# tomvanbraeckel/amv-codec-tools

Measured on AMD Instinct MI355X. Metric: AMV frames/sec/GPU (160x120 decode, bit-exact), higher is better.
Workload: dtype int32; 1 GPU; 160x120 AMV decode, 160000-frame synthetic stream per GPU, chunks resident in HBM; parallelism=frame-range x1, frames_per_gpu=160000, stream=seeded synthetic source (BASELINE.md section 4), every frame

## Files before the change

### amv-codec-tools_amd/csrc/amv_reconstruct.hip

```cpp
#include "amv_block_load.h"

namespace amv {

namespace {

struct __attribute__((aligned(4))) Px12 { uint32_t w[3]; };

constexpr int kRowsPerGroup = 4;

__device__ __forceinline__ int mad24(int x, int w, int c) {
    int d;
    asm("v_mad_i32_i24 %0, %1, %2, %3" : "=v"(d) : "v"(x), "s"(w), "v"(c));
    return d;
}

enum RowKind { kRowPlain, kRow0, kRow4 };

template <bool kColumn, RowKind kKind = kRowPlain>
__device__ __forceinline__ void idct8(int& v0, int& v1, int& v2, int& v3, int& v4, int& v5, int& v6, int& v7) {
    constexpr int W1 = 2841, W2 = 2676, W3 = 2408, W5 = 1609, W6 = 1108, W7 = 565;
    constexpr int kBias = kKind == kRow0 ? 128 + 8192 : 128;
    constexpr int kRound = kColumn ? 4 : 0;
    constexpr int kDown = kColumn ? 3 : 0;
    constexpr int kOut = kColumn ? 14 : 8;
    int a0 = kColumn ? v0 : v0 * 2048 + kBias, a1 = kColumn ? v4 : v4 * 2048;
    const int i2 = v6, i3 = v2, i4 = v1, i5 = v7, i6 = v5, i7 = v3;
    int t;
    int a4 = mad24(i4, W1, mad24(i5, W7, kRound)) >> kDown;
    int a5 = mad24(i4, W7, mad24(i5, -W1, kRound)) >> kDown;
    int a6 = mad24(i6, W5, mad24(i7, W3, kRound)) >> kDown;
    int a7 = mad24(i6, W3, mad24(i7, -W5, kRound)) >> kDown;
    t = a0 + a1;
    a0 -= a1;
    int a2 = mad24(i3, W6, mad24(i2, -W2, kRound)) >> kDown;
    int a3 = mad24(i3, W2, mad24(i2, W6, kRound)) >> kDown;
    a1 = a4 + a6;
    a4 -= a6;
    a6 = a5 + a7;
    a5 -= a7;
    a7 = t + a3;
    t -= a3;
    a3 = a0 + a2;
    a0 -= a2;
    a2 = (181 * (a4 + a5) + 128) >> 8;
    a4 = (181 * (a4 - a5) + 128) >> 8;
    v0 = a7 + a1;
    v1 = a3 + a2;
    v2 = a0 + a4;
    v3 = t + a6;
    v4 = t - a6;
    v5 = a0 - a4;
    v6 = a3 - a2;
    v7 = a7 - a1;
    if (kKind == kRowPlain) {
        v0 >>= kOut; v1 >>= kOut; v2 >>= kOut; v3 >>= kOut; v4 >>= kOut; v5 >>= kOut; v6 >>= kOut; v7 >>= kOut;
    } else {
        v0 &= ~255; v1 &= ~255; v2 &= ~255; v3 &= ~255; v4 &= ~255; v5 &= ~255; v6 &= ~255; v7 &= ~255;
    }
}

struct QuantWords { uint32_t w[2][16]; };
constexpr QuantWords pack_quant() {
    QuantWords q{};
    for (int i = 0; i < 64; ++i) {
        q.w[0][i >> 2] |= (uint32_t)kQuantLuma[i] << (8 * (i & 3));
        q.w[1][i >> 2] |= (uint32_t)kQuantChroma[i] << (8 * (i & 3));
    }
    return q;
}
__device__ const QuantWords kQuantWords = pack_quant();

__device__ __forceinline__ int clamp_iclp(int x) { return min(max(x, -256), 255); }

constexpr uint32_t pair16(int lo, int hi) { return ((uint32_t)lo & 0xffffu) | ((uint32_t)hi << 16); }
__device__ __forceinline__ uint32_t dot2_bias(uint32_t a, uint32_t w) {
    uint32_t d;
    asm("v_dot2_i32_i16 %0, %1, %2, %3" : "=v"(d) : "v"(a), "s"(w), "v"(32768u));
    return d;
}

__device__ __forceinline__ uint32_t sat_pair(uint32_t yy, uint32_t cc) {
    uint32_t sum, d;
    asm("v_pk_add_i16 %0, %1, %2" : "=v"(sum) : "v"(yy), "v"(cc));
    asm("v_sat_pk_u8_i16 %0, %1" : "=v"(d) : "v"(sum));
    return d;
}

}

template <bool kRound, int kRows>
__global__ __launch_bounds__(kWave * kRows) void amv_reconstruct_kernel(
    SyncSinks in, const uint32_t* __restrict__ nmcu_ok, uint32_t n, FrameSel sel,
    FrameGeom g, PieceMap pm, uint32_t flags, uint8_t* __restrict__ out) {
    constexpr uint32_t kPitchY = kSegMcus * 16, kPitchC = kSegMcus * 8;
    __shared__ __attribute__((aligned(16))) int16_t s_all[kRows][16 * kPitchY + 2 * 8 * kPitchC + 64];
    static_assert((16 * kPitchY + 2 * 8 * kPitchC) * 2 == kSegImageBytes, "the planes reuse the image");
    const uint32_t lane = threadIdx.x & 63u, wave = (uint32_t)__builtin_amdgcn_readfirstlane((int)(threadIdx.x >> 6));
    uint32_t item, row_group, seg;
    if (!locate_piece(pm, blockIdx.x, item, row_group, seg)) return;
    const uint32_t my = row_group * kRows + wave;
    if (my >= g.mcu_rows) return;
    int16_t* const s_mem = s_all[wave];
    int16_t* const s_y = s_mem;
    int16_t* const s_u = s_mem + 16 * kPitchY;
    int16_t* const s_v = s_u + 8 * kPitchC;
    uint8_t* const s_img = reinterpret_cast<uint8_t*>(s_mem);

    uint32_t qw[16];
    {
        const uint4* q4 = reinterpret_cast<const uint4*>(kQuantWords.w[lane % 6u >= 4u ? 1 : 0]);
#pragma unroll
        for (int i = 0; i < 4; ++i) {
            const uint4 q = q4[i];
            qw[4 * i] = q.x; qw[4 * i + 1] = q.y; qw[4 * i + 2] = q.z; qw[4 * i + 3] = q.w;
        }
    }
    do {
    uint32_t f, slot;
    if (!select_frame(sel, n, item, f, slot)) return;
    const Segment sg = segment_of(f, slot, nmcu_ok, g, pm.nseg, my, seg);
    const uint32_t m0 = sg.m0, cnt = sg.cnt, ok = sg.ok, mcu0 = sg.mcu0;

    uint32_t c[32];
    bool skip;
    if (load_segment_blocks(in, sg, kRound, g, lane, s_img, c, skip)) {
        const uint32_t m = lane / 6u, k6 = lane % 6u;
        const bool chroma = k6 >= 4u;
        int v[64];
#pragma unroll
        for (int nat = 0; nat < 64; ++nat) {
            const int scan = kScanOfNatural[nat];
            v[nat] = coef_at(c, scan) * (int)((qw[scan >> 2] >> (8 * (scan & 3))) & 255u);
        }
        if (!(flags & kFlagZigzagFixed))
            v[kAmvlibQuirkNatural] = coef_at(c, kAmvlibQuirkScan) * (int)((qw[kAmvlibQuirkScan >> 2] >> (8 * (kAmvlibQuirkScan & 3))) & 255u);
#pragma unroll
        for (int r = 0; r < 8; ++r) {
            if (r == 0) idct8<false, kRow0>(v[0], v[1], v[2], v[3], v[4], v[5], v[6], v[7]);
            else if (r == 4) idct8<false, kRow4>(v[32], v[33], v[34], v[35], v[36], v[37], v[38], v[39]);
            else idct8<false>(v[8 * r], v[8 * r + 1], v[8 * r + 2], v[8 * r + 3], v[8 * r + 4], v[8 * r + 5], v[8 * r + 6], v[8 * r + 7]);
        }
#pragma unroll
        for (int col = 0; col < 8; ++col)
            idct8<true>(v[col], v[8 + col], v[16 + col], v[24 + col], v[32 + col], v[40 + col], v[48 + col], v[56 + col]);
        int16_t* dst = chroma ? (k6 == 4u ? s_u : s_v) + m * 8u
                              : s_y + ((k6 >> 1) * 8u) * kPitchY + m * 16u + (k6 & 1u) * 8u;
        const uint32_t pitch = chroma ? kPitchC : kPitchY;
#pragma unroll
        for (int r = 0; r < 8; ++r) {
            uint32_t w[4];
#pragma unroll
            for (int q = 0; q < 4; ++q) {
                const int lo = clamp_iclp(v[8 * r + 2 * q]);
                const int hi = clamp_iclp(v[8 * r + 2 * q + 1]);
                w[q] = __builtin_amdgcn_perm((uint32_t)hi, (uint32_t)lo, 0x05040100u);
            }
            *reinterpret_cast<uint4*>(dst + r * pitch) = make_uint4(w[0], w[1], w[2], w[3]);
        }
    }
    if (skip) return;
    seg_sync();

    const uint32_t vr = min(16u, g.height - my * 16u);
    const uint32_t px = min(cnt * 16u, g.width - m0 * 16u);
    const uint32_t groups = cnt * 4u;
    const bool all_decoded = mcu0 + cnt <= ok;
    const uint32_t pairs = (vr + 1u) >> 1;
    const uint32_t step_i2 = kWave / groups, step_gi = kWave - step_i2 * groups;
    uint32_t i2 = lane / groups, gi = lane - i2 * groups;
    uint8_t* const frame = out + (uint64_t)f * g.frame_bytes;
    const uint32_t row0 = (g.height - 1u - my * 16u) * g.stride + m0 * 48u;
    for (; i2 < pairs; i2 += step_i2, gi += step_gi) {
        if (gi >= groups) { gi -= groups; ++i2; if (i2 >= pairs) break; }
        const uint32_t lc = gi * 4u;
        uint2 ya = *reinterpret_cast<const uint2*>(s_y + (2u * i2) * kPitchY + lc);
        uint2 yb = *reinterpret_cast<const uint2*>(s_y + (2u * i2 + 1u) * kPitchY + lc);
        uint32_t uu = *reinterpret_cast<const uint32_t*>(s_u + i2 * kPitchC + (lc >> 1));
        uint32_t vv = *reinterpret_cast<const uint32_t*>(s_v + i2 * kPitchC + (lc >> 1));
        if (!all_decoded && (mcu0 + (gi >> 2)) >= ok) {
            constexpr uint32_t kDark = 0xfc00fc00u;
            ya.x = ya.y = yb.x = yb.y = kDark;
            uu = vv = 0u;
        }
        uint32_t cr[2], cg[2], cb[2];
#pragma unroll
        for (int e = 0; e < 2; ++e) {
            const uint32_t uv = __builtin_amdgcn_perm(vv, uu, e ? 0x07060302u : 0x05040100u);
            const uint32_t r = dot2_bias(uv, pair16(18, 367));
            const uint32_t gg = dot2_bias(uv, pair16(-159, -220));
            const uint32_t b = dot2_bias(uv, pair16(411, -29));
            cr[e] = __builtin_amdgcn_perm(r, r, 0x02010201u);
            cg[e] = __builtin_amdgcn_perm(gg, gg, 0x02010201u);
            cb[e] = __builtin_amdgcn_perm(b, b, 0x02010201u);
        }
        if (lc >= px) continue;
        uint32_t off = row0 - 2u * i2 * g.stride + lc * 3u;
#pragma unroll
        for (int row = 0; row < 2; ++row) {
            const uint2 yy = row ? yb : ya;
            const uint32_t b01 = sat_pair(yy.x, cb[0]), g01 = sat_pair(yy.x, cg[0]), r01 = sat_pair(yy.x, cr[0]);
            const uint32_t b23 = sat_pair(yy.y, cb[1]), g23 = sat_pair(yy.y, cg[1]), r23 = sat_pair(yy.y, cr[1]);
            const uint32_t gr = g01 | (r01 << 16);
            const uint32_t bg = b23 | (g23 << 16);
            Px12 v;
            v.w[0] = __builtin_amdgcn_perm(gr, b01, 0x01060400u);
            v.w[1] = __builtin_amdgcn_perm(bg, gr, 0x06040301u);
            v.w[2] = __builtin_amdgcn_perm(bg, r23, 0x01070500u);
            if (2u * i2 + (uint32_t)row >= vr) break;
            if (lc + 4u <= px) {
                *reinterpret_cast<Px12*>(frame + off) = v;
            } else {
#pragma unroll
                for (uint32_t q = 0; q < 9u; ++q)
                    if (q < (px - lc) * 3u) frame[off + q] = (uint8_t)(v.w[q >> 2] >> (8u * (q & 3u)));
            }
            off -= g.stride;
        }
    }
    } while (next_item<kRound>(pm, item));
}

template <int kRows, class... Args>
static void launch_rows(const FrameGeom& g, Args... args) {
    launch_segments(amv_reconstruct_kernel<false, kRows>, amv_reconstruct_kernel<true, kRows>, kWave * kRows, (g.mcu_rows + kRows - 1) / kRows, args...);
}

void launch_reconstruct(const SyncSinks& sinks, const uint32_t* nmcu_ok, uint32_t n, const FrameSel& sel, uint32_t items,
                        const FrameGeom& g, uint32_t flags, uint8_t* out, hipStream_t s) {
    const uint32_t slots4 = (g.mcu_rows + 3u) / 4u * 4u, slots5 = (g.mcu_rows + 4u) / 5u * 5u;
    const uint32_t waste4 = slots4 - g.mcu_rows, waste5 = slots5 - g.mcu_rows;
    if (10u * waste4 * slots5 >= 10u * waste5 * slots4 + slots4 * slots5) launch_rows<5>(g, sinks, nmcu_ok, n, sel, items, g, s, flags, out);
    else launch_rows<kRowsPerGroup>(g, sinks, nmcu_ok, n, sel, items, g, s, flags, out);
}

__global__ __launch_bounds__(kWave * 4) void amv_expand_records_kernel(SyncSinks in, const uint32_t* __restrict__ nmcu_ok, uint32_t n,
                                                                        FrameGeom g, uint32_t nseg, int16_t* __restrict__ coef) {
    __shared__ __attribute__((aligned(16))) uint8_t s_img[4][kSegImageBytes + 128];
    const uint32_t lane = threadIdx.x & 63u, wave = threadIdx.x >> 6;
    const uint32_t segs = g.mcu_rows * nseg;
    const uint64_t pairs = (uint64_t)n * segs;
    for (uint64_t p = (uint64_t)blockIdx.x * 4u + wave; p < pairs; p += (uint64_t)gridDim.x * 4u) {
        const uint32_t f = (uint32_t)(p / segs), segidx = (uint32_t)(p % segs);
        const Segment sg = segment_of(f, f, nmcu_ok, g, nseg, segidx / nseg, segidx % nseg);
        uint32_t c[32];
        bool skip;
        if (load_segment_blocks(in, sg, false, g, lane, s_img[wave], c, skip)) {
            const uint32_t blk = sg.mcu0 * 6u + lane;
            if (blk >= (in.ok_in_blocks ? sg.ok : sg.ok * 6u)) {
#pragma unroll
                for (int i = 0; i < 32; ++i) c[i] = 0u;
            }
            uint4* d = reinterpret_cast<uint4*>(coef + ((uint64_t)f * g.blocks + blk) * 64u);
#pragma unroll
            for (int i = 0; i < 8; ++i) d[i] = make_uint4(c[4 * i], c[4 * i + 1], c[4 * i + 2], c[4 * i + 3]);
        }
        seg_sync();
    }
}

void launch_expand_records(const SyncSinks& sinks, const uint32_t* nmcu_ok, uint32_t n, const FrameGeom& g, int16_t* coef,
                           hipStream_t s) {
    const uint32_t nseg = segs_per_row(g);
    const uint64_t groups = ((uint64_t)n * g.mcu_rows * nseg + 3u) / 4u;
    if (groups == 0) return;
    hipLaunchKernelGGL(amv_expand_records_kernel, dim3(groups < 65536u ? (uint32_t)groups : 65536u), dim3(kWave * 4), 0, s, sinks,
                       nmcu_ok, n, g, nseg, coef);
}

}
```

Measured before the change: 29.65 million frames/s.

## Add fully-unrolled fast path for full segments and packed IDCT clamp

```diff
diff --git a/amv-codec-tools_amd/csrc/amv_reconstruct.hip b/amv-codec-tools_amd/csrc/amv_reconstruct.hip
--- a/amv-codec-tools_amd/csrc/amv_reconstruct.hip
+++ b/amv-codec-tools_amd/csrc/amv_reconstruct.hip
@@ -22,7 +22,7 @@
     constexpr int kBias = kKind == kRow0 ? 128 + 8192 : 128;
     constexpr int kRound = kColumn ? 4 : 0;
     constexpr int kDown = kColumn ? 3 : 0;
-    constexpr int kOut = kColumn ? 14 : 8;
+    constexpr int kOut = kColumn ? 7 : 8;
     int a0 = kColumn ? v0 : v0 * 2048 + kBias, a1 = kColumn ? v4 : v4 * 2048;
     const int i2 = v6, i3 = v2, i4 = v1, i5 = v7, i6 = v5, i7 = v3;
     int t;
@@ -70,7 +70,12 @@
 }
 __device__ const QuantWords kQuantWords = pack_quant();
 
-__device__ __forceinline__ int clamp_iclp(int x) { return min(max(x, -256), 255); }
+__device__ __forceinline__ uint32_t clamp_pack(int lo, int hi) {
+    uint32_t p, d;
+    asm("v_cvt_pk_i16_i32 %0, %1, %2" : "=v"(p) : "v"(lo), "v"(hi));
+    asm("v_pk_ashrrev_i16 %0, %1, %2" : "=v"(d) : "s"(0x00070007u), "v"(p));
+    return d;
+}
 
 constexpr uint32_t pair16(int lo, int hi) { return ((uint32_t)lo & 0xffffu) | ((uint32_t)hi << 16); }
 __device__ __forceinline__ uint32_t dot2_bias(uint32_t a, uint32_t w) {
@@ -84,6 +89,33 @@
     asm("v_pk_add_i16 %0, %1, %2" : "=v"(sum) : "v"(yy), "v"(cc));
     asm("v_sat_pk_u8_i16 %0, %1" : "=v"(d) : "v"(sum));
     return d;
+}
+
+struct ChromaTerms { uint32_t r[2], g[2], b[2]; };
+__device__ __forceinline__ ChromaTerms chroma_terms(uint32_t uu, uint32_t vv) {
+    ChromaTerms c;
+#pragma unroll
+    for (int e = 0; e < 2; ++e) {
+        const uint32_t uv = __builtin_amdgcn_perm(vv, uu, e ? 0x07060302u : 0x05040100u);
+        const uint32_t r = dot2_bias(uv, pair16(18, 367));
+        const uint32_t gg = dot2_bias(uv, pair16(-159, -220));
+        const uint32_t b = dot2_bias(uv, pair16(411, -29));
+        c.r[e] = __builtin_amdgcn_perm(r, r, 0x02010201u);
+        c.g[e] = __builtin_amdgcn_perm(gg, gg, 0x02010201u);
+        c.b[e] = __builtin_amdgcn_perm(b, b, 0x02010201u);
+    }
+    return c;
+}
+__device__ __forceinline__ Px12 patch_row(uint2 yy, const ChromaTerms& c) {
+    const uint32_t b01 = sat_pair(yy.x, c.b[0]), g01 = sat_pair(yy.x, c.g[0]), r01 = sat_pair(yy.x, c.r[0]);
+    const uint32_t b23 = sat_pair(yy.y, c.b[1]), g23 = sat_pair(yy.y, c.g[1]), r23 = sat_pair(yy.y, c.r[1]);
+    const uint32_t gr = g01 | (r01 << 16);
+    const uint32_t bg = b23 | (g23 << 16);
+    Px12 v;
+    v.w[0] = __builtin_amdgcn_perm(gr, b01, 0x01060400u);
+    v.w[1] = __builtin_amdgcn_perm(bg, gr, 0x06040301u);
+    v.w[2] = __builtin_amdgcn_perm(bg, r23, 0x01070500u);
+    return v;
 }
 
 }
@@ -150,11 +182,7 @@
         for (int r = 0; r < 8; ++r) {
             uint32_t w[4];
 #pragma unroll
-            for (int q = 0; q < 4; ++q) {
-                const int lo = clamp_iclp(v[8 * r + 2 * q]);
-                const int hi = clamp_iclp(v[8 * r + 2 * q + 1]);
-                w[q] = __builtin_amdgcn_perm((uint32_t)hi, (uint32_t)lo, 0x05040100u);
-            }
+            for (int q = 0; q < 4; ++q) w[q] = clamp_pack(v[8 * r + 2 * q], v[8 * r + 2 * q + 1]);
             *reinterpret_cast<uint4*>(dst + r * pitch) = make_uint4(w[0], w[1], w[2], w[3]);
         }
     }
@@ -165,11 +193,38 @@
     const uint32_t px = min(cnt * 16u, g.width - m0 * 16u);
     const uint32_t groups = cnt * 4u;
     const bool all_decoded = mcu0 + cnt <= ok;
+    uint8_t* const frame = out + (uint64_t)f * g.frame_bytes;
+    const uint32_t row0 = (g.height - 1u - my * 16u) * g.stride + m0 * 48u;
+    constexpr uint32_t kPairY = 4u * kPitchY, kPairC = 2u * kPitchC, kPlaneU = 32u * kPitchY, kPlaneV = kPlaneU + 16u * kPitchC;
+    if (all_decoded && cnt == kSegMcus && px == kSegMcus * 16u && vr == 16u) {
+        constexpr uint32_t kGroups = kSegMcus * 4u, kTrips = kGroups * 8u / kWave;
+        static_assert(kGroups * 8u % kWave == 0u && kGroups < kWave && kPairC == kGroups * 4u, "whole trips; chroma is linear in t");
+        const uint32_t a = lane >= kGroups ? 1u : 0u, b = lane - a * kGroups;
+        const uint8_t* const ly = s_img + a * kPairY + b * 8u;
+        const uint8_t* const ly_past = ly + (kPairY - kGroups * 8u);
+        const uint8_t* const lc = s_img + kPlaneU + lane * 4u;
+        const uint32_t off0 = row0 - a * 2u * g.stride + b * 12u;
+        const uint32_t off0_past = off0 - 2u * g.stride - kGroups * 12u;
+#pragma unroll
+        for (uint32_t k = 0; k < kTrips; ++k) {
+            const uint32_t q = k * kWave / kGroups, r = k * kWave % kGroups;
+            const bool past = r != 0u && b >= kGroups - r;
+            const uint8_t* const y = (past ? ly_past : ly) + (q * kPairY + r * 8u);
+            const uint2 ya = *reinterpret_cast<const uint2*>(y);
+            const uint2 yb = *reinterpret_cast<const uint2*>(y + 2u * kPitchY);
+            const uint32_t uu = *reinterpret_cast<const uint32_t*>(lc + k * kWave * 4u);
+            const uint32_t vv = *reinterpret_cast<const uint32_t*>(lc + k * kWave * 4u + (kPlaneV - kPlaneU));
+            const ChromaTerms c = chroma_terms(uu, vv);
+            uint8_t* const upper = frame + (int64_t)(int32_t)(r * 12u - q * 2u * g.stride);
+            const uint32_t off = past ? off0_past : off0;
+            *reinterpret_cast<Px12*>(upper + off) = patch_row(ya, c);
+            *reinterpret_cast<Px12*>(upper - g.stride + off) = patch_row(yb, c);
+        }
+        continue;
+    }
     const uint32_t pairs = (vr + 1u) >> 1;
     const uint32_t step_i2 = kWave / groups, step_gi = kWave - step_i2 * groups;
     uint32_t i2 = lane / groups, gi = lane - i2 * groups;
-    uint8_t* const frame = out + (uint64_t)f * g.frame_bytes;
-    const uint32_t row0 = (g.height - 1u - my * 16u) * g.stride + m0 * 48u;
     for (; i2 < pairs; i2 += step_i2, gi += step_gi) {
         if (gi >= groups) { gi -= groups; ++i2; if (i2 >= pairs) break; }
         const uint32_t lc = gi * 4u;
@@ -182,30 +237,12 @@
             ya.x = ya.y = yb.x = yb.y = kDark;
             uu = vv = 0u;
         }
-        uint32_t cr[2], cg[2], cb[2];
-#pragma unroll
-        for (int e = 0; e < 2; ++e) {
-            const uint32_t uv = __builtin_amdgcn_perm(vv, uu, e ? 0x07060302u : 0x05040100u);
-            const uint32_t r = dot2_bias(uv, pair16(18, 367));
-            const uint32_t gg = dot2_bias(uv, pair16(-159, -220));
-            const uint32_t b = dot2_bias(uv, pair16(411, -29));
-            cr[e] = __builtin_amdgcn_perm(r, r, 0x02010201u);
-            cg[e] = __builtin_amdgcn_perm(gg, gg, 0x02010201u);
-            cb[e] = __builtin_amdgcn_perm(b, b, 0x02010201u);
-        }
+        const ChromaTerms c = chroma_terms(uu, vv);
         if (lc >= px) continue;
         uint32_t off = row0 - 2u * i2 * g.stride + lc * 3u;
 #pragma unroll
         for (int row = 0; row < 2; ++row) {
-            const uint2 yy = row ? yb : ya;
-            const uint32_t b01 = sat_pair(yy.x, cb[0]), g01 = sat_pair(yy.x, cg[0]), r01 = sat_pair(yy.x, cr[0]);
-            const uint32_t b23 = sat_pair(yy.y, cb[1]), g23 = sat_pair(yy.y, cg[1]), r23 = sat_pair(yy.y, cr[1]);
-            const uint32_t gr = g01 | (r01 << 16);
-            const uint32_t bg = b23 | (g23 << 16);
-            Px12 v;
-            v.w[0] = __builtin_amdgcn_perm(gr, b01, 0x01060400u);
-            v.w[1] = __builtin_amdgcn_perm(bg, gr, 0x06040301u);
-            v.w[2] = __builtin_amdgcn_perm(bg, r23, 0x01070500u);
+            const Px12 v = patch_row(row ? yb : ya, c);
             if (2u * i2 + (uint32_t)row >= vr) break;
             if (lc + 4u <= px) {
                 *reinterpret_cast<Px12*>(frame + off) = v;
```

New measurement: 30.83 million frames/s (median of 6 runs). +4.0%, better.
